# sashapersonxyz/Multi-camera_3D_Pose_Estimation

Measured on AMD Instinct MI355X. Metric: multi-view frames/sec end-to-end (2-cam HRNet-W32, 17 kpts) at 1/2/4/8 GPUs, higher is better.
Workload: dtype bf16; 1 GPU; BASELINE config 2: 2-cam HRNet-W32 256x192 bf16 (flip test) + batched 4x4 DLT-SVD triangulation; views=2, parallelism=dp1 (frame-sharded)

## Files before the change

### include/mvpose.h

```cpp
#ifndef MVPOSE_H
#define MVPOSE_H

#include <stddef.h>
#include <stdint.h>

#ifdef __cplusplus
extern "C" {
#endif

#define MVP_ABI_VERSION 1

#define MVP_OK 0
#define MVP_ERR_ARG (-1)
#define MVP_ERR_HIP (-2)
#define MVP_ERR_NOMEM (-3)
#define MVP_ERR_INTERNAL (-4)

int mvp_abi_version(void);
const char* mvp_last_error(void);

#define MVP_CAM_DOUBLES 40

int mvp_camera_pack(const double* K_host, const double* dist5_host, const double* R_host,
                    const double* T_host, double* out_record_host);
// ... 49 lines not shown

#define MVP_OP_STEM 0
#define MVP_OP_CONV 1
#define MVP_OP_FUSE 2

typedef struct mvp_tensor_desc {
    int h, w, c, dtype;
} mvp_tensor_desc;

typedef struct mvp_op_desc {
    int kind;
    int out;
    int n_in;
    int in[4];
    int up[4];
    int cin, cout, ks, stride, relu;
    int segment;
    int64_t w_off;
    int64_t b_off;
} mvp_op_desc;

int mvp_graph_create(const mvp_tensor_desc* tensors_host, int n_tensors, const mvp_op_desc* ops_host, int n_ops,
                     const int* seg_micro_batch_host, int n_segments, int input_tensor, int output_tensor,
                     const uint16_t* w_bf16_dev, int64_t w_elems, const float* f32_dev, int64_t f32_elems,
                     int max_batch, void** handle_out);
int mvp_graph_forward(void* handle, const void* input_dev, int batch, void* output_dev, void* stream);
int mvp_graph_arena_bytes(void* handle, int64_t* bytes_out);
int mvp_graph_refresh_weights(void* handle);
int mvp_graph_destroy(void* handle);
int mvp_graph_plan(void* handle, int batch, int64_t* rec_out, int max_records, int* n_records,
                   int64_t* covered_macs_out);
int mvp_graph_kernels(void* handle, int batch, int* kernels_out, int max_records, int* n_records);
const char* mvp_graph_kernel_name(int kernel);

#define MVP_DET_STEM 0
#define MVP_DET_CONV 1
#define MVP_DET_DW 2
#define MVP_DET_CA 3
#define MVP_DET_SPP 4
#define MVP_DET_UP2 5
#define MVP_DET_HEAD 6
#define MVP_DET_DWPW 7

typedef struct mvp_det_view {
    int t;
    int coff;
    int c;
} mvp_det_view;

typedef struct mvp_det_op {
    int kind;
    mvp_det_view in, out, res;
    int ks, stride, act;
    int64_t w_off, b_off;
    int64_t aux;
} mvp_det_op;

int mvp_det_letterbox(const uint8_t* frames_dev, int n, int h, int w, int size, const float* mean3_host,
                      const float* std3_host, void* out_dev, void* stream);
int mvp_det_create(const mvp_tensor_desc* tensors_host, int n_tensors, const mvp_det_op* ops_host, int n_ops,
                   int input_tensor, int size, int n_priors, const uint16_t* w_bf16_dev, int64_t w_elems,
                   const float* f32_dev, int64_t f32_elems, int max_batch, void** handle_out);
int mvp_det_forward(void* handle, const uint8_t* frames_dev, int n, int h, int w, float score_thr, float* cand_dev,
                    float* best_dev, void* letterboxed_dev, void* stream);
int mvp_det_nms(const float* cand_dev, int n, int n_priors, const int* level_off_host, int n_levels, int nms_pre,
                float score_thr, float iou_thr, int max_det, float fx, float fy, float* dets_dev, int* counts_dev,
// ... 147 lines not shown
```

### multi-camera_3d_pose_estimation_amd/csrc/conv.h

```cpp
#pragma once
#include <hip/hip_runtime.h>
#include <cstdint>

#include "kernel_select.h"
#include "mvp_common.h"

namespace mvp {

struct ConvLaunch {
    const uint16_t* x;
    const uint16_t* w;
    const float* bias;
    const uint16_t* res;
    uint16_t* y;
    float* yf;
    int N, H, W, Cin, Cout;
    int ks, stride, relu, out_f32_nchw;
    const uint16_t* x2 = nullptr;
    int c1 = 0;
    int x_stride = 0, y_stride = 0, r_stride = 0;
    const uint16_t* w_img = nullptr;
    int s2_tile = 0;
};


void launch_conv_generic(const ConvLaunch& c, hipStream_t s);

void launch_head1x1(const ConvLaunch& c, hipStream_t s);
bool head_fuse_supported(int cin, int cout, int n_in);
void launch_head_fuse(const uint16_t* const* in, const int* up, int n_in, int relu, const uint16_t* w,
                      const float* bias, float* y, int N, int H, int W, hipStream_t s);

void launch_conv1x1_direct(const ConvLaunch& c, hipStream_t s);
void launch_conv1x1_wide(const ConvLaunch& c, hipStream_t s);

struct PairLaunch {
    const uint16_t* x = nullptr;
    const uint16_t* x2 = nullptr;
    int c1 = 0, c2 = 0;
    const uint16_t* w1 = nullptr;
    const float* b1 = nullptr;
    const uint16_t* res = nullptr;
    uint16_t* y = nullptr;
    const uint16_t* w2 = nullptr;
    const float* b2 = nullptr;
    uint16_t* y2 = nullptr;
    long n_pix = 0;
};
bool conv1x1_pair_supported(int cin_total, int cmid, int cout2);
void launch_conv1x1_pair(const PairLaunch& p, hipStream_t s);


struct BneckLaunch {
    const uint16_t* x = nullptr;
    const uint16_t* w1 = nullptr;
    const float* b1 = nullptr;
    const uint16_t* w2 = nullptr;
    const float* b2 = nullptr;
    const uint16_t* w3 = nullptr;
    const float* b3 = nullptr;
    uint16_t* y = nullptr;
    int N = 0, H = 0, W = 0;
    int perm = 1;
    int lead = 0;
    int planar = 0;
};
bool bneck_supported(int H, int W, int C, int M);
void launch_bneck(const BneckLaunch& c, hipStream_t s);

void launch_tconv(const ConvLaunch& c, hipStream_t s);
void launch_tconv16(const ConvLaunch& c, hipStream_t s);
void tconv16_pack_weights(const uint16_t* w, uint16_t* img, int cin, int cout, hipStream_t s);

void launch_s2conv(const ConvLaunch& c, hipStream_t s);

struct S2Multi {
    const uint16_t* x = nullptr;
    const uint16_t* w = nullptr;
    const float* bias = nullptr;
    int N = 0, H = 0, W = 0, Cin = 0;
    int n_out = 0;
    uint16_t* y[3] = {nullptr, nullptr, nullptr};
    int cout[3] = {0, 0, 0};
    int relu[3] = {0, 0, 0};
};
bool s2conv_multi_supported(int H, int W, int Cin, int total_cout);
void launch_s2conv_multi(const S2Multi& m, hipStream_t s);

void launch_stem(const uint16_t* x, const float* w, const float* bias, uint16_t* y, int N, int H, int W,
                 hipStream_t s);

bool stem2_supported(int H, int W, int cin2, int cout2);
void launch_stem2(const uint16_t* x, const float* w1, const float* b1, const uint16_t* w2, const float* b2,
                  uint16_t* y, int N, int H, int W, bool crop_ranges, hipStream_t s);

bool trans1_supported(int H, int W, int C, int cout0, int cout1);
void launch_trans1(const uint16_t* x, const uint16_t* wimg, const float* b0, const float* b1, uint16_t* y0,
                   uint16_t* y1, int N, bool planar, hipStream_t s);
constexpr long kTrans1ImageElems = 16L * 9 * 2 * 96 * 8;
void trans1_pack_weights(const uint16_t* wb, int64_t w0_off, int64_t w1_off, uint16_t* img, hipStream_t s);

void launch_fuse_sum(const uint16_t* const* in, const int* up, int n_in, uint16_t* out, int N, int H, int W,
                     int C, int relu, hipStream_t s);

constexpr int kZeroSlots = 4096;
const uint16_t* conv_zero_region();
uint16_t* conv_sink_region();

template <auto Kern, int LDS, typename... Args>
void launch_lds(int grid, int threads, hipStream_t s, const Args&... args) {
    static const bool attr = [] {
        MVP_HIP(hipFuncSetAttribute((const void*)Kern, hipFuncAttributeMaxDynamicSharedMemorySize, LDS));
        return true;
    }();
    (void)attr;
    hipLaunchKernelGGL(Kern, dim3(grid), dim3(threads), LDS, s, args...);
}
// ... 14 lines not shown
```

### multi-camera_3d_pose_estimation_amd/csrc/graph.cpp

```cpp
#include <algorithm>
#include <cstdlib>
#include <cstring>
#include <vector>

#include "conv.h"
#include "mvp_common.h"

namespace mvp {
namespace {

struct Launch {
    Route route;
    int op;
    std::vector<int> covers;
    std::vector<int> reads;
    std::vector<int> writes;
    KernelChoice kernel;
    int64_t macs = 0;
    int cat_src = -1;
    int tail = -1;
    int conv1 = -1, conv2 = -1;
    int perm = 0;
    int lead = 0;
    int stem = -1;
// ... 24 lines not shown
    int cus = 0;
    std::vector<Launch> launches;
    std::vector<int> owner;
    std::vector<int64_t> offset;
    int64_t arena_bytes = 0;
    char* arena = nullptr;
};

int64_t elem_size(int dtype) { return dtype == MVP_DT_F32_NCHW ? 4 : 2; }

int64_t tensor_bytes(const mvp_tensor_desc& t, int batch) {
    return (int64_t)batch * t.h * t.w * t.c * elem_size(t.dtype);
}

Switches read_switches() {
    auto first_is = [](const char* name, char c) {
        const char* e = getenv(name);
        return e && e[0] == c;
    };
    Switches sw;
    sw.no_fuse = first_is("MVPOSE_NO_FUSE", '1');
    sw.no_catfuse = first_is("MVPOSE_NO_CATFUSE", '1');
    sw.no_pairfuse = first_is("MVPOSE_NO_PAIRFUSE", '1');
    sw.no_bneck = first_is("MVPOSE_NO_BNECK", '1');
    sw.no_stemfuse = first_is("MVPOSE_NO_STEMFUSE", '1');
    sw.no_transfuse = first_is("MVPOSE_NO_TRANSFUSE", '1');
    sw.no_sibfuse = first_is("MVPOSE_NO_SIBFUSE", '1');
    sw.no_headfuse = first_is("MVPOSE_NO_HEADFUSE", '1');
    sw.no_tblock64 = first_is("MVPOSE_NO_TBLOCK64", '1');
    sw.no_head1x1 = first_is("MVPOSE_NO_HEAD1X1", '1');
    sw.no_tconv = first_is("MVPOSE_NO_TCONV", '1');
    sw.no_tconv16 = first_is("MVPOSE_TCONV16", '0');
    sw.no_s2conv = first_is("MVPOSE_NO_S2CONV", '1');
    sw.no_tblock = first_is("MVPOSE_NO_TBLOCK", '1');
    sw.no_tblock32s = first_is("MVPOSE_NO_TBLOCK32S", '1');
    sw.stem2_tile = first_is("MVPOSE_STEM2_TILE", '1');
    sw.crop_stream = first_is("MVPOSE_CROP_STREAM", '1');
    const char* e = getenv("MVPOSE_S2_TILE");
    sw.s2_tile = e ? atoi(e) : 0;
    return sw;
}

void validate(Graph& g, int64_t w_elems, int64_t f_elems) {
    const int nt = (int)g.tensors.size();
    auto T = [&](int id) -> const mvp_tensor_desc& {
        MVP_REQUIRE(id >= 0 && id < nt, "graph: tensor id %d out of range", id);
        return g.tensors[id];
    };
    std::vector<int> defined(nt, 0);
    defined[g.input] = 1;
    for (size_t k = 0; k < g.ops.size(); k++) {
        const mvp_op_desc& op = g.ops[k];
        const mvp_tensor_desc& o = T(op.out);
        MVP_REQUIRE(op.n_in >= 1 && op.n_in <= 4, "graph op %zu: n_in=%d", k, op.n_in);
        for (int i = 0; i < op.n_in; i++) {
            if (op.kind == MVP_OP_CONV && i == 1 && op.in[1] < 0) continue;
            T(op.in[i]);
            MVP_REQUIRE(defined[op.in[i]], "graph op %zu reads tensor %d before it is produced", k, op.in[i]);
        }
        MVP_REQUIRE(!defined[op.out], "graph op %zu: tensor %d produced twice", k, op.out);
        if (op.kind == MVP_OP_STEM) {
            const mvp_tensor_desc& x = T(op.in[0]);
            MVP_REQUIRE(x.c == 4 && x.dtype == MVP_DT_BF16_NHWC, "stem: input must be bf16 NHWC with 4 channels");
            MVP_REQUIRE(o.c == 64 && o.h == (x.h - 1) / 2 + 1 && o.w == (x.w - 1) / 2 + 1, "stem: output shape");
            MVP_REQUIRE(op.w_off >= 0 && op.w_off + 64 * 36 <= f_elems && op.b_off >= 0 && op.b_off + 64 <= f_elems,
                        "stem: weights out of the f32 blob");
// ... 598 lines not shown
        const mvp_op_desc& op = g->ops[L.op];
        const mvp_tensor_desc& o = g->tensors[op.out];
        const mvp_tensor_desc& x = g->tensors[L.reads[0]];
        const mvp::Kernel kernel = mvp::pick_kernel(L.kernel, nb, g->cus, g->sw);
        switch (L.route) {
        case mvp::R_BLOCK: {
            const mvp_op_desc& c1 = g->ops[L.op - 1];
            const uint16_t *xb = bf16(op.in[1]), *w1 = g->wb + c1.w_off, *w2 = g->wb + op.w_off;
            const float *b1 = g->fb + c1.b_off, *b2 = g->fb + op.b_off;
            uint16_t* y = bf16(op.out);
            switch (kernel) {
            case mvp::K_TBLOCK32S: mvp::launch_tblock32s(xb, w1, b1, w2, b2, y, nb, o.h, o.w, s); break;
            case mvp::K_TBLOCK32: mvp::launch_tblock32(xb, w1, b1, w2, b2, y, nb, o.h, o.w, s); break;
            case mvp::K_BASIC_BLOCK_C32: mvp::launch_basic_block_c32(xb, w1, b1, w2, b2, y, nb, o.h, o.w, s); break;
            default: mvp::launch_tblock64(xb, w1, b1, w2, b2, y, nb, o.h, o.w, kernel == mvp::K_TBLOCK64, s);
            }
            break;
        }
        case mvp::R_TWIN: {
            const mvp_op_desc& b = g->ops[L.twin];
            mvp::launch_trans1(bf16(op.in[0]), L.w_img, g->fb + op.b_off, g->fb + b.b_off, bf16(op.out),
                               bf16(b.out), nb, L.planar, s);
            break;
        }
        case mvp::R_SIBLINGS: {
            mvp::S2Multi m;
            m.x = bf16(op.in[0]), m.w = L.w, m.bias = L.b;
            m.N = nb, m.H = x.h, m.W = x.w, m.Cin = op.cin;
            m.n_out = (int)L.covers.size();
            for (int i = 0; i < m.n_out; i++) {
                const mvp_op_desc& o2 = g->ops[L.covers[i]];
                m.y[i] = bf16(o2.out), m.cout[i] = o2.cout, m.relu[i] = o2.relu;
            }
            mvp::launch_s2conv_multi(m, s);
            break;
        }
        case mvp::R_HEAD_FUSE: {
            const mvp_op_desc& f = g->ops[L.fuse];
            const mvp_tensor_desc& fo = g->tensors[f.out];
            const uint16_t* ins[4];
            for (int i = 0; i < f.n_in; i++) ins[i] = bf16(f.in[i]);
            mvp::launch_head_fuse(ins, f.up, f.n_in, f.relu, g->wb + op.w_off, g->fb + op.b_off, (float*)ptr(op.out),
                                  nb, fo.h, fo.w, s);
            break;
        }
        case mvp::R_BNECK: {
            const mvp_op_desc& a = g->ops[L.conv1];
            const mvp_op_desc& c2 = g->ops[L.conv2];
            mvp::BneckLaunch bl;
            bl.x = bf16(a.in[0]);
            bl.w1 = g->wb + a.w_off, bl.b1 = g->fb + a.b_off;
            bl.w2 = g->wb + c2.w_off, bl.b2 = g->fb + c2.b_off;
            bl.w3 = L.lead ? L.w : g->wb + op.w_off, bl.b3 = L.lead ? L.b : g->fb + op.b_off;
            bl.y = bf16(op.out);
            bl.N = nb, bl.H = x.h, bl.W = x.w;
            bl.perm = L.perm, bl.lead = L.lead, bl.planar = L.planar;
            mvp::launch_bneck(bl, s);
            break;
        }
        case mvp::R_STEM2: {
            const mvp_op_desc& st = g->ops[L.stem];
            mvp::launch_stem2(bf16(st.in[0]), g->fb + st.w_off, g->fb + st.b_off, g->wb + op.w_off, g->fb + op.b_off,
                              bf16(op.out), nb, x.h, x.w, kernel == mvp::K_STEM2, s);
            break;
        }
        case mvp::R_STEM:
            mvp::launch_stem(bf16(op.in[0]), g->fb + op.w_off, g->fb + op.b_off, bf16(op.out), nb, x.h, x.w, s);
            break;
        case mvp::R_CONV:
        case mvp::R_PAIR: {
            mvp::ConvLaunch c{};
            c.x = bf16(op.in[0]);
            c.w = g->wb + op.w_off, c.bias = g->fb + op.b_off;
            c.res = mvp::has_res(op) ? bf16(op.in[1]) : nullptr;
            c.out_f32_nchw = o.dtype == MVP_DT_F32_NCHW;
            c.y = c.out_f32_nchw ? nullptr : bf16(op.out);
            c.yf = c.out_f32_nchw ? (float*)ptr(op.out) : nullptr;
            c.N = nb, c.H = x.h, c.W = x.w;
            c.Cin = op.cin, c.Cout = op.cout, c.ks = op.ks, c.stride = op.stride, c.relu = op.relu;
            c.w_img = L.w_img, c.s2_tile = g->sw.s2_tile;
            if (L.cat_src >= 0) {
                const mvp_op_desc& a = g->ops[L.cat_src];
                c.x2 = bf16(a.in[0]), c.c1 = op.cin, c.Cin = op.cin + a.cin;
                c.w = L.w, c.bias = L.b, c.res = nullptr;
            }
            if (L.route == mvp::R_CONV) {
                switch (kernel) {
                case mvp::K_HEAD1X1: mvp::launch_head1x1(c, s); break;
                case mvp::K_CONV1X1_WIDE: mvp::launch_conv1x1_wide(c, s); break;
                case mvp::K_CONV1X1: mvp::launch_conv1x1_direct(c, s); break;
                case mvp::K_TCONV: mvp::launch_tconv(c, s); break;
                case mvp::K_TCONV16: mvp::launch_tconv16(c, s); break;
                case mvp::K_S2CONV: mvp::launch_s2conv(c, s); break;
                default: mvp::launch_conv_generic(c, s);
                }
                break;
            }
            const mvp_op_desc& b = g->ops[L.tail];
            mvp::PairLaunch pl;
            pl.x = c.x, pl.x2 = c.x2;
            pl.c1 = c.x2 ? c.c1 : c.Cin, pl.c2 = c.x2 ? c.Cin - c.c1 : 0;
            pl.w1 = c.w, pl.b1 = c.bias, pl.res = c.res, pl.y = c.y;
            pl.w2 = g->wb + b.w_off, pl.b2 = g->fb + b.b_off, pl.y2 = bf16(b.out);
            pl.n_pix = (long)nb * x.h * x.w;
            mvp::launch_conv1x1_pair(pl, s);
            break;
        }
        case mvp::R_FUSE_SUM: {
            const uint16_t* ins[4];
            for (int i = 0; i < op.n_in; i++) ins[i] = bf16(op.in[i]);
            mvp::launch_fuse_sum(ins, op.up, op.n_in, bf16(op.out), nb, o.h, o.w, o.c, op.relu, s);
            break;
        }
// ... 14 lines not shown
    MVP_REQUIRE(batch > 0 && batch <= g->max_batch, "mvp_graph_plan: batch %d", batch);
    int n = 0;
    int64_t total = 0;
    mvp::for_each_micro_batch(*g, batch, [&](const mvp::Segment& sg, int64_t, int nb) {
        for (int l = sg.first_launch; l < sg.end_launch; l++, n++) {
            const Launch& L = g->launches[l];
            total += L.macs * nb;
            if (n >= max_records) continue;
            const int64_t rec[4] = {L.op, L.route, nb, L.macs * nb};
            std::copy(rec, rec + 4, rec_out + 4 * n);
        }
    });
    *n_records = n;
    if (covered_macs_out) *covered_macs_out = total;
    MVP_ABI_END
}

extern "C" int mvp_graph_kernels(void* handle, int batch, int* kernels_out, int max_records, int* n_records) {
    MVP_ABI_BEGIN
    Graph* g = static_cast<Graph*>(handle);
    MVP_REQUIRE(g && kernels_out && n_records, "mvp_graph_kernels: NULL pointer");
    MVP_REQUIRE(batch > 0 && batch <= g->max_batch, "mvp_graph_kernels: batch %d", batch);
    int n = 0;
    mvp::for_each_micro_batch(*g, batch, [&](const mvp::Segment& sg, int64_t, int nb) {
        for (int l = sg.first_launch; l < sg.end_launch; l++, n++)
            if (n < max_records) kernels_out[n] = mvp::pick_kernel(g->launches[l].kernel, nb, g->cus, g->sw);
    });
    *n_records = n;
    MVP_ABI_END
}

extern "C" const char* mvp_graph_kernel_name(int kernel) { return mvp::kernel_name(kernel); }

extern "C" int mvp_graph_refresh_weights(void* handle) {
    MVP_ABI_BEGIN
    Graph* g = static_cast<Graph*>(handle);
    MVP_REQUIRE(g != nullptr, "mvp_graph_refresh_weights: NULL handle");
    MVP_HIP(hipDeviceSynchronize());
    mvp::fill_weights(*g);
    MVP_ABI_END
}

extern "C" int mvp_graph_arena_bytes(void* handle, int64_t* bytes_out) {
    MVP_ABI_BEGIN
    MVP_REQUIRE(handle && bytes_out, "mvp_graph_arena_bytes: NULL argument");
    *bytes_out = static_cast<Graph*>(handle)->arena_bytes;
    MVP_ABI_END
}

extern "C" int mvp_graph_destroy(void* handle) {
    MVP_ABI_BEGIN
    Graph* g = static_cast<Graph*>(handle);
    if (g) {
        if (g->arena) (void)hipFree(g->arena);
        mvp::free_weights(*g);
        delete g;
    }
    MVP_ABI_END
}
```

### multi-camera_3d_pose_estimation_amd/csrc/kernel_select.h

```cpp
#pragma once

namespace mvp {

struct Switches {
    bool no_fuse = false;
    bool no_catfuse = false;
    bool no_pairfuse = false;
    bool no_bneck = false;
    bool no_stemfuse = false;
    bool no_transfuse = false;
    bool no_sibfuse = false;
    bool no_headfuse = false;
    bool no_tblock64 = false;
    bool no_head1x1 = false;
    bool no_tconv = false;
    bool no_tconv16 = false;
    bool no_s2conv = false;
    bool no_tblock = false;
    bool no_tblock32s = false;
    bool stem2_tile = false;
    bool crop_stream = false;
    int s2_tile = 0;
};

enum Route {
    R_BLOCK = 1,
    R_TWIN = 2,
    R_SIBLINGS = 3,
    R_HEAD_FUSE = 4,
    R_BNECK = 5,
    R_STEM2 = 6,
    R_STEM = 7,
    R_CONV = 8,
    R_PAIR = 9,
    R_FUSE_SUM = 10,
};

enum Kernel {
    K_NONE = 0,
    K_HEAD1X1,
    K_CONV1X1_WIDE,
    K_CONV1X1,
    K_TCONV,
    K_TCONV16,
    K_S2CONV,
    K_CONV_MFMA,
    K_TBLOCK32S,
    K_TBLOCK32,
    K_BASIC_BLOCK_C32,
    K_TBLOCK64,
// ... 68 lines not shown
    if (plane && c.stride == 2 && !c.res && !sw.no_s2conv) {
        if (c.h == 64 && c.w == 48 && c.cout == 64 && c.cin == 32) return K_S2CONV;
        if (c.h == 32 && c.w == 24 && c.cout == 128 && (c.cin == 32 || c.cin == 64)) return K_S2CONV;
        if (s2conv_streams_image(c)) return K_S2CONV;
    }
    return K_CONV_MFMA;
}

inline KernelChoice select_kernel(Route route, const LaunchShape& c, const Switches& sw, bool has_image) {
    auto one = [](Kernel k) { return KernelChoice{k, k}; };
    switch (route) {
    case R_CONV: return one(select_conv(c, sw, has_image));
    case R_BLOCK: {
        if (c.cin == 64) return {K_TBLOCK64_TILES, K_TBLOCK64};
        const Kernel tile = c.w == 48 && c.h % 16 == 0 && !sw.no_tblock ? K_TBLOCK32 : K_BASIC_BLOCK_C32;
        const bool s32 = c.h == 64 && c.w == 48 && !sw.no_tblock32s && !sw.no_tblock;
        return {tile, s32 ? K_TBLOCK32S : tile};
    }
    case R_STEM2: return {K_STEM2_TILE, sw.stem2_tile ? K_STEM2_TILE : K_STEM2};
    case R_STEM: {
        const int ho = (c.h - 1) / 2 + 1, wo = (c.w - 1) / 2 + 1;
        return one(wo == 96 && c.h % 2 == 0 && ho % 2 == 0 ? K_STEM_MFMA : K_STEM);
    }
    case R_TWIN: return one(K_TRANS1);
    case R_SIBLINGS: return one(K_S2CONV_MULTI);
    case R_HEAD_FUSE: return one(K_HEAD_FUSE);
    case R_BNECK: return one(K_BNECK);
    case R_PAIR: return one(K_CONV1X1_PAIR);
    case R_FUSE_SUM: return one(K_FUSE_SUM);
    }
    return {};
}

inline long conv_image_elems(Kernel k, const LaunchShape& c) {
    return k == K_TCONV16 || (k == K_S2CONV && s2conv_streams_image(c)) ? (long)c.cout * 9 * c.cin : 0;
}

}
```

### multi-camera_3d_pose_estimation_amd/csrc/s2conv.hip

```cpp
#include <algorithm>
#include <cstdlib>

#include "conv.h"
#include "mfma_tile.h"
#include "mvp_common.h"

namespace mvp {
namespace {

using namespace mfma_tile;

template <int CIN, int H, int W, int TH, int NB, bool WRES, int BM>
struct SCfg {
    static constexpr int NW = 8, NT_THREADS = NW * 64;
    static constexpr int MG = BM / 32, PG = NW / MG;
    static constexpr int NT = 3;
    static constexpr int HO = H / 2, WO = W / 2;
    static constexpr int P = NB * TH * WO;
    static constexpr int NCH = CIN / 16;
    static constexpr int RS = WO + 1, HR = TH + 1;
    static constexpr int PH = HR * RS;
    static constexpr int HS = NB * 4 * PH;
    static constexpr int HT = 2 * HS;
    static constexpr int QS = 1, PS = 2;
    static constexpr int WT = 9 * 2 * BM;
    static constexpr int ITEM_SLOTS = HT + (WRES ? 0 : WT);
    static constexpr int PPW = (ITEM_SLOTS + 64 * NW - 1) / (64 * NW);
    static constexpr int BUF = PPW * NW * 1024;
    static constexpr int WPPW = WRES ? (NCH * WT + 64 * NW - 1) / (64 * NW) : 0;
    static constexpr int WOFF = 2 * BUF;
    static constexpr int LDS = 2 * BUF + WPPW * NW * 1024;
    static constexpr int STORES = 2 * NT;
    static_assert(P == PG * NT * 32, "tile = pixel groups x 3 fragments x 32 pixels");
    static_assert(H % 2 == 0 && W % 2 == 0 && HO % TH == 0 && CIN % 16 == 0, "tiling");
    static_assert(LDS <= 160 * 1024, "LDS budget");
    static_assert((QS + (3 * PH + RS + 1) * PS) * 16 < 65536 && (16 * BM + 2 * BM) * 16 < 65536,
                  "ds_read offset range");
    static_assert(STORES < 64 && 2 * PPW < 64, "vmcnt range");
// ... 150 lines not shown
            const int cur = tap & 1;
            if (tap + 1 < 9) load(tap + 1, fa[cur ^ 1], fb[cur ^ 1]);
            __builtin_amdgcn_sched_barrier(0);
#pragma unroll
            for (int t = 0; t < G::NT; t++)
                acc[t] = __builtin_amdgcn_mfma_f32_32x32x16_bf16(fa[cur], fb[cur][t], acc[t], 0, 0, 0);
            __builtin_amdgcn_sched_barrier(0);
        }

        if (last) {
            const long pix0 = (long)(n0 * G::HO + ho0) * G::WO;
            uint16_t* yb = p.y;
            int cs = p.Cout, cl = cob, rl = p.relu;
            bool cok = true;
            if (cob >= p.Cout) {
                const bool s1 = cob < p.Cout + p.c1;
                yb = s1 ? p.y1 : p.y2;
                cs = s1 ? p.c1 : p.c2;
                cl = s1 ? cob - p.Cout : cob - p.Cout - p.c1;
                rl = s1 ? p.relu1 : p.relu2;
                cok = cob < p.Cout + p.c1 + p.c2;
            }
#pragma unroll
            for (int t = 0; t < G::NT; t++) {
                const bool ok = n0 + enb[t] < p.N && cok;
                uint16_t* yrow = ok ? yb + (pix0 + eoff[t]) * cs + cl : p.sink + lane * 16;
                store_row16(yrow, pack_row16(acc[t], rl != 0));
            }
        }
    }
    asm volatile("s_waitcnt vmcnt(0)" ::: "memory");
}

template <int CIN, int H, int W, int TH, int NB, bool WRES, int BM>
void launch_sp(const SParams& p, hipStream_t s) {
    using G = SCfg<CIN, H, W, TH, NB, WRES, BM>;
    const int grid = std::min(p.n_tiles, cu_count());
    launch_lds<s2conv_kernel<CIN, H, W, TH, NB, WRES, BM>, G::LDS>(grid, G::NT_THREADS, s, p);
}

template <int CIN, int H, int W, int TH, int NB, bool WRES, int BM>
void launch_s(const ConvLaunch& c, hipStream_t s) {
    using G = SCfg<CIN, H, W, TH, NB, WRES, BM>;
    MVP_REQUIRE(!WRES || c.Cout == BM, "s2conv: resident weights need Cout == BM");
    MVP_REQUIRE(c.Cout % BM == 0, "s2conv: Cout %d not a multiple of %d", c.Cout, BM);
    MVP_REQUIRE(c.Cin == CIN && c.H == H && c.W == W, "s2conv: plane mismatch");
    const long tiles = (long)((c.N + NB - 1) / NB) * (G::HO / TH) * (c.Cout / BM);
    MVP_REQUIRE(tiles < (1L << 30), "s2conv: too many tiles");
    const bool img = !WRES && BM == 128 && c.w_img != nullptr;
    SParams p{c.x, img ? c.w_img : c.w, c.bias, c.y, conv_zero_region(), conv_sink_region(), c.N, c.Cout, (int)tiles,
              c.Cout / BM, c.relu, nullptr, nullptr, 0, 0, 0, 0, img ? 1 : 0};
    launch_sp<CIN, H, W, TH, NB, WRES, BM>(p, s);
}

}

bool s2conv_multi_supported(int H, int W, int Cin, int total_cout) {
    return H == 64 && W == 48 && Cin == 32 && total_cout <= 128;
}

void launch_s2conv_multi(const S2Multi& m, hipStream_t s) {
    MVP_REQUIRE(m.n_out >= 1 && m.n_out <= 3, "s2conv_multi: %d outputs", m.n_out);
    int tot = 0;
    for (int i = 0; i < m.n_out; i++) {
        MVP_REQUIRE(m.cout[i] % 32 == 0 && m.cout[i] > 0, "s2conv_multi: cout %d", m.cout[i]);
        tot += m.cout[i];
    }
    MVP_REQUIRE(s2conv_multi_supported(m.H, m.W, m.Cin, tot), "s2conv_multi: unsupported plane");
    using G = SCfg<32, 64, 48, 8, 1, true, 128>;
    const long tiles = (long)m.N * (G::HO / 8);
    SParams p{m.x, m.w, m.bias, m.y[0], conv_zero_region(), conv_sink_region(), m.N, m.cout[0], (int)tiles, 1, m.relu[0],
              m.n_out > 1 ? m.y[1] : nullptr, m.n_out > 2 ? m.y[2] : nullptr, m.n_out > 1 ? m.cout[1] : 0,
              m.n_out > 2 ? m.cout[2] : 0, m.n_out > 1 ? m.relu[1] : 0, m.n_out > 2 ? m.relu[2] : 0, 0};
    if (tiles == 0) return;
    launch_sp<32, 64, 48, 8, 1, true, 128>(p, s);
    MVP_HIP(hipGetLastError());
}

void launch_s2conv(const ConvLaunch& c, hipStream_t s) {
    MVP_REQUIRE(c.ks == 3 && c.stride == 2 && !c.out_f32_nchw && !c.res && !c.x2, "s2conv: not a plain 3x3/s2 conv");
    const int ci = c.Cin, co = c.Cout, h = c.H, w = c.W;
    const bool p24 = h == 32 && w == 24 && co == 128;
    const bool p12 = h == 16 && w == 12 && co % 128 == 0;
    if (h == 64 && w == 48 && co == 64 && ci == 32)
        launch_s<32, 64, 48, 16, 1, true, 64>(c, s);
    else if (p24 && ci == 32)
        launch_s<32, 32, 24, 16, 1, true, 128>(c, s);
    else if (p24 && ci == 64)
        launch_s<64, 32, 24, 16, 1, false, 128>(c, s);
    else if (p12 && ci == 32)
        launch_s<32, 16, 12, 8, 4, false, 128>(c, s);
    else if (p12 && ci == 64)
        launch_s<64, 16, 12, 8, 4, false, 128>(c, s);
    else if (p12 && ci == 128)
        launch_s<128, 16, 12, 8, 4, false, 128>(c, s);
    else
        fail(MVP_ERR_ARG, "s2conv: unsupported plane %d -> %d @ %dx%d", ci, co, h, w);
    MVP_HIP(hipGetLastError());
}

}
```

### multi-camera_3d_pose_estimation_amd/mvpose/_lib.py

```python
from __future__ import annotations

import ctypes
import os

_HERE = os.path.dirname(os.path.abspath(__file__))
LIB_PATH = os.environ.get("MVPOSE_LIB", os.path.join(_HERE, "libmvpose.so"))


class MvposeError(RuntimeError):

    def __init__(self, fn: str, code: int, msg: str):
        super().__init__(f"{fn} failed (code {code}): {msg}")
        self.code = code


if not os.path.exists(LIB_PATH):
    raise ImportError(
        f"libmvpose.so not found at {LIB_PATH}: build it with "
        "`make -C multi-camera_3d_pose_estimation_amd` (or __graft_entry__.build()). "
        "There is no CPU fallback.")

lib = ctypes.CDLL(LIB_PATH)

c_int, c_int64, c_float, c_double, c_void_p, c_size_t = (
# ... 13 lines not shown
                                       c_int, c_void_p, c_int, c_float, c_float, c_int, c_double, c_void_p,
                                       c_void_p, c_void_p, c_void_p, c_void_p]),
    "mvp_triangulate_points_f64": (c_int, [c_void_p, c_int64, c_void_p, c_void_p, c_void_p, c_void_p]),
    "mvp_triangulate_fallback_total": (c_int, [c_void_p, P(ctypes.c_ulonglong)]),
    "mvp_mp4v_create": (c_int, [c_void_p, c_size_t, P(c_void_p), P(c_int), P(c_int)]),
    "mvp_mp4v_decode": (c_int, [c_void_p, c_void_p, c_size_t, c_void_p, c_void_p, P(c_int)]),
    "mvp_mp4v_destroy": (c_int, [c_void_p]),
    "mvp_mp4v_selfcheck": (c_int, []),
    "mvp_mp4v_parse": (c_int, [c_void_p, c_void_p, c_size_t, c_void_p, c_int64, c_void_p, c_int64, P(c_int64),
                               P(c_int)]),
    "mvp_mp4v_reconstruct": (c_int, [c_void_p, c_int, c_int, c_int, c_void_p]),
    "mvp_mp4v_parse_many": (c_int, [c_void_p, c_int, c_void_p, c_void_p, c_void_p, c_void_p, c_int64, c_void_p,
                                    c_void_p, P(c_int)]),
    "mvp_preprocess": (c_int, [c_void_p, c_int, c_int, c_int, c_void_p, c_int, c_int, P(c_float), P(c_float),
                               c_int, c_int, c_void_p, c_void_p]),
    "mvp_heatmap_decode": (c_int, [c_void_p, c_void_p, c_int, c_int, c_int, c_int, P(c_int), c_int, c_void_p,
                                   c_int, c_int, c_void_p, c_void_p, c_void_p, c_void_p, c_void_p, c_int,
                                   c_void_p]),
    "mvp_warp_is_separable": (c_int, [P(c_double), c_int, c_int, P(c_int)]),
    "mvp_heatmap_revert": (c_int, [c_void_p, c_int, c_int, c_int, c_int, c_void_p, c_int, c_int, c_void_p,
                                   c_void_p]),
    "mvp_heatmap_moments": (c_int, [c_void_p, c_int, c_int, c_int, c_int, c_void_p, c_int, c_int, c_float,
                                    c_int, c_void_p, c_void_p, c_void_p]),
    "mvp_bbox_geometry": (c_int, [c_void_p, c_int, c_int, c_int, c_float, c_int, c_int, c_void_p, c_void_p,
                                  c_void_p, c_void_p, c_void_p]),
    "mvp_graph_create": (c_int, None),
    "mvp_graph_forward": (c_int, [c_void_p, c_void_p, c_int, c_void_p, c_void_p]),
    "mvp_graph_arena_bytes": (c_int, None),
    "mvp_graph_refresh_weights": (c_int, [c_void_p]),
    "mvp_graph_destroy": (c_int, [c_void_p]),
    "mvp_graph_plan": (c_int, [c_void_p, c_int, c_void_p, c_int, P(c_int), P(c_int64)]),
    "mvp_graph_kernels": (c_int, [c_void_p, c_int, c_void_p, c_int, P(c_int)]),
    "mvp_graph_kernel_name": (c_char_p, [c_int]),
    "mvp_det_letterbox": (c_int, [c_void_p, c_int, c_int, c_int, c_int, P(c_float), P(c_float), c_void_p,
                                  c_void_p]),
    "mvp_det_create": (c_int, None),
    "mvp_det_forward": (c_int, [c_void_p, c_void_p, c_int, c_int, c_int, c_float, c_void_p, c_void_p, c_void_p,
                                c_void_p]),
    "mvp_det_nms": (c_int, [c_void_p, c_int, c_int, P(c_int), c_int, c_int, c_float, c_float, c_int, c_float,
                            c_float, c_void_p, c_void_p, c_void_p]),
    "mvp_det_arena_bytes": (c_int, None),
    "mvp_det_run_ops": (c_int, [c_void_p, c_void_p, c_int, c_int, c_int, c_int, c_int, c_void_p, c_void_p]),
    "mvp_det_tensor_copy": (c_int, [c_void_p, c_int, c_int, c_void_p, c_int, c_void_p]),
    "mvp_det_folded_ops": (c_int, [c_void_p, c_void_p, c_int]),
    "mvp_det_kernels": (c_int, [c_void_p, c_void_p, c_int, P(c_int)]),
    "mvp_det_kernel_name": (c_char_p, [c_int]),
    "mvp_det_destroy": (c_int, [c_void_p]),
    "mvp_sgd_workspace_floats": (c_int, [c_int, c_int, c_int, c_int, P(c_int64)]),
    "mvp_sgd_refine": (c_int, None),
    "mvp_sgd_refine_cams": (c_int, None),
    "mvp_extrinsic_sample_grad": (c_int, [c_void_p, c_void_p, c_int, c_int64, c_void_p, c_int, c_int, c_void_p,
                                          c_void_p]),
    "mvp_extrinsic_adam_step": (c_int, [c_void_p, c_int, c_void_p, c_void_p, c_double, c_double, c_double, c_double,
                                        c_double, c_void_p, c_void_p, c_void_p]),
    "mvp_project_points": (c_int, [c_void_p, c_int64, c_void_p, c_int, c_void_p, c_void_p]),
    "mvp_linear_interpolation": (c_int, [c_void_p, c_int, c_int, c_int, c_int, c_float, c_float, c_int, c_int,
                                         c_void_p, c_void_p]),
    "mvp_trajectory_smooth_plan": (c_int, [c_int, c_int, c_int, P(c_int), P(c_int), P(c_int64)]),
    "mvp_trajectory_smooth": (c_int, [c_void_p, c_void_p, c_void_p, c_int, c_int, c_double, c_float, c_float, c_int,
                                      c_void_p, c_int64, c_void_p, c_void_p, c_void_p, c_void_p, c_void_p]),
    "mvp_trajectory_smooth_cov_plan": (c_int, [c_int, c_int, c_int, P(c_int), P(c_int), P(c_int64)]),
    "mvp_trajectory_smooth_cov": (c_int, [c_void_p, c_void_p, c_void_p, c_int, c_int, c_double, c_float, c_float,
                                          c_int, c_void_p, c_int64, c_void_p, c_void_p, c_void_p, c_void_p]),
    "mvp_epipolar_lag_cost_plan": (c_int, [c_int, c_int, c_int, c_int, P(c_int), P(c_int64)]),
    "mvp_epipolar_lag_cost": (c_int, [c_void_p, c_int, c_int, c_int, c_void_p, c_int, P(c_int), c_int, c_int, c_float,
                                      c_float, c_void_p, c_int64, c_void_p, c_void_p, c_void_p]),
# ... 59 lines not shown
```

### multi-camera_3d_pose_estimation_amd/mvpose/hrnet.py

```python
from __future__ import annotations

import ctypes
import os

import numpy as np
import torch

from . import _lib
from ._lib import call

BN_EPS = 1e-5
STAGES = ((1, (32, 64)), (4, (32, 64, 128)), (3, (32, 64, 128, 256)))
N_JOINTS = 17
INPUT_HW = (256, 192)
HEATMAP_HW = (64, 48)
DT_BF16, DT_F32 = 0, 1
OP_STEM, OP_CONV, OP_FUSE = 0, 1, 2


class TensorDesc(ctypes.Structure):
    _fields_ = [("h", ctypes.c_int), ("w", ctypes.c_int), ("c", ctypes.c_int), ("dtype", ctypes.c_int)]


class OpDesc(ctypes.Structure):
# ... 504 lines not shown
        world, _ = mdist.world_rank()
        if world > 1:
            mdist.broadcast_([self.w_dev, self.f_dev], src=src)
            torch.cuda.synchronize(self.device)
            self.refresh_weights()

    @property
    def arena_bytes(self) -> int:
        b = ctypes.c_int64()
        call("mvp_graph_arena_bytes", self._h, ctypes.byref(b))
        return b.value

    def launch_plan(self, batch: int) -> np.ndarray:
        cap = 4096
        rec = np.zeros((cap, 4), np.int64)
        n, tot = ctypes.c_int(), ctypes.c_int64()
        call("mvp_graph_plan", self._h, int(batch), ctypes.c_void_p(rec.ctypes.data), cap, ctypes.byref(n),
             ctypes.byref(tot))
        if n.value > cap:
            raise RuntimeError(f"{n.value} launches > {cap}")
        rec = rec[:n.value].copy()
        assert int(rec[:, 3].sum()) == tot.value == self.macs_per_crop() * batch
        return rec

    def launch_kernels(self, batch: int) -> list[str]:
        cap = 4096
        ids = np.zeros(cap, np.int32)
        n = ctypes.c_int()
        call("mvp_graph_kernels", self._h, int(batch), ctypes.c_void_p(ids.ctypes.data), cap, ctypes.byref(n))
        if n.value > cap:
            raise RuntimeError(f"{n.value} launches > {cap}")
        return [_lib.lib.mvp_graph_kernel_name(int(k)).decode() for k in ids[:n.value]]

    def macs_per_crop(self) -> int:
        macs = 0
        for op in self.spec.ops:
            if op["kind"] in (OP_STEM, OP_CONV):
                h, w, _, _ = self.spec.tensors[op["out"]]
                cin = 3 if op["kind"] == OP_STEM else op["cin"]
                macs += h * w * op["cout"] * cin * op["ks"] ** 2
        return macs

    def close(self):
        if getattr(self, "_h", None):
            call("mvp_graph_destroy", self._h)
            self._h = None

    def __del__(self):
        try:
            self.close()
        except Exception:
            pass


class HRNetBackbone(ConvGraph):

    def __init__(self, state_dict=None, seed: int = 0, max_batch: int = 256, device="cuda", micro_batch=None):
        if state_dict is None:
            state_dict = random_state_dict(seed)
        spec, input_id, output_id = build_hrnet_w32(state_dict, micro_batch)
        super().__init__(spec, input_id, output_id, max_batch, device)

    def forward(self, crops: torch.Tensor, out: torch.Tensor | None = None) -> torch.Tensor:
        if crops.dtype != torch.bfloat16 or not crops.is_cuda or not crops.is_contiguous():
            raise ValueError("crops must be a contiguous bf16 CUDA tensor (N,256,192,4)")
        if tuple(crops.shape[1:]) != (INPUT_HW[0], INPUT_HW[1], 4):
# ... 8 lines not shown
```

Measured before the change: 13040 frames/s.

## Add halo-tiled persistent stride-2 conv kernel with double-buffered LDS staging

```diff
diff --git a/include/mvpose.h b/include/mvpose.h
--- a/include/mvpose.h
+++ b/include/mvpose.h
@@ -105,6 +105,7 @@
                    int64_t* covered_macs_out);
 int mvp_graph_kernels(void* handle, int batch, int* kernels_out, int max_records, int* n_records);
 const char* mvp_graph_kernel_name(int kernel);
+int mvp_graph_s2conv_forms(void* handle, int batch, int* forms_out, int max_records, int* n_records);
 
 #define MVP_DET_STEM 0
 #define MVP_DET_CONV 1
diff --git a/multi-camera_3d_pose_estimation_amd/csrc/conv.h b/multi-camera_3d_pose_estimation_amd/csrc/conv.h
--- a/multi-camera_3d_pose_estimation_amd/csrc/conv.h
+++ b/multi-camera_3d_pose_estimation_amd/csrc/conv.h
@@ -21,6 +21,7 @@
     int x_stride = 0, y_stride = 0, r_stride = 0;
     const uint16_t* w_img = nullptr;
     int s2_tile = 0;
+    int s2_items = 0;
 };
 
 
@@ -83,6 +84,7 @@
     uint16_t* y[3] = {nullptr, nullptr, nullptr};
     int cout[3] = {0, 0, 0};
     int relu[3] = {0, 0, 0};
+    int items = 0;
 };
 bool s2conv_multi_supported(int H, int W, int Cin, int total_cout);
 void launch_s2conv_multi(const S2Multi& m, hipStream_t s);
diff --git a/multi-camera_3d_pose_estimation_amd/csrc/graph.cpp b/multi-camera_3d_pose_estimation_amd/csrc/graph.cpp
--- a/multi-camera_3d_pose_estimation_amd/csrc/graph.cpp
+++ b/multi-camera_3d_pose_estimation_amd/csrc/graph.cpp
@@ -80,6 +80,7 @@
     sw.no_tconv = first_is("MVPOSE_NO_TCONV", '1');
     sw.no_tconv16 = first_is("MVPOSE_TCONV16", '0');
     sw.no_s2conv = first_is("MVPOSE_NO_S2CONV", '1');
+    sw.s2conv_items = first_is("MVPOSE_S2CONV_ITEMS", '1');
     sw.no_tblock = first_is("MVPOSE_NO_TBLOCK", '1');
     sw.no_tblock32s = first_is("MVPOSE_NO_TBLOCK32S", '1');
     sw.stem2_tile = first_is("MVPOSE_STEM2_TILE", '1');
@@ -744,6 +745,7 @@
                 const mvp_op_desc& o2 = g->ops[L.covers[i]];
                 m.y[i] = bf16(o2.out), m.cout[i] = o2.cout, m.relu[i] = o2.relu;
             }
+            m.items = g->sw.s2conv_items;
             mvp::launch_s2conv_multi(m, s);
             break;
         }
@@ -790,7 +792,7 @@
             c.yf = c.out_f32_nchw ? (float*)ptr(op.out) : nullptr;
             c.N = nb, c.H = x.h, c.W = x.w;
             c.Cin = op.cin, c.Cout = op.cout, c.ks = op.ks, c.stride = op.stride, c.relu = op.relu;
-            c.w_img = L.w_img, c.s2_tile = g->sw.s2_tile;
+            c.w_img = L.w_img, c.s2_tile = g->sw.s2_tile, c.s2_items = g->sw.s2conv_items;
             if (L.cat_src >= 0) {
                 const mvp_op_desc& a = g->ops[L.cat_src];
                 c.x2 = bf16(a.in[0]), c.c1 = op.cin, c.Cin = op.cin + a.cin;
@@ -871,6 +873,23 @@
 
 extern "C" const char* mvp_graph_kernel_name(int kernel) { return mvp::kernel_name(kernel); }
 
+extern "C" int mvp_graph_s2conv_forms(void* handle, int batch, int* forms_out, int max_records, int* n_records) {
+    MVP_ABI_BEGIN
+    Graph* g = static_cast<Graph*>(handle);
+    MVP_REQUIRE(g && forms_out && n_records, "mvp_graph_s2conv_forms: NULL pointer");
+    MVP_REQUIRE(batch > 0 && batch <= g->max_batch, "mvp_graph_s2conv_forms: batch %d", batch);
+    int n = 0;
+    mvp::for_each_micro_batch(*g, batch, [&](const mvp::Segment& sg, int64_t, int nb) {
+        for (int l = sg.first_launch; l < sg.end_launch; l++, n++) {
+            if (n >= max_records) continue;
+            const Launch& L = g->launches[l];
+            forms_out[n] = mvp::s2conv_form(mvp::pick_kernel(L.kernel, nb, g->cus, g->sw), mvp::launch_shape(*g, L), g->sw);
+        }
+    });
+    *n_records = n;
+    MVP_ABI_END
+}
+
 extern "C" int mvp_graph_refresh_weights(void* handle) {
     MVP_ABI_BEGIN
     Graph* g = static_cast<Graph*>(handle);
diff --git a/multi-camera_3d_pose_estimation_amd/csrc/kernel_select.h b/multi-camera_3d_pose_estimation_amd/csrc/kernel_select.h
--- a/multi-camera_3d_pose_estimation_amd/csrc/kernel_select.h
+++ b/multi-camera_3d_pose_estimation_amd/csrc/kernel_select.h
@@ -16,6 +16,7 @@
     bool no_tconv = false;
     bool no_tconv16 = false;
     bool no_s2conv = false;
+    bool s2conv_items = false;
     bool no_tblock = false;
     bool no_tblock32s = false;
     bool stem2_tile = false;
@@ -150,6 +151,23 @@
     return {};
 }
 
+enum S2Form {
+    S2_NONE = 0,
+    S2_ITEMS = 1,
+    S2_HALO = 2,
+};
+
+inline bool s2conv_halo_plane(int cin, int cout, int h, int w) {
+    if (h == 64 && w == 48) return cin == 32 && (cout == 64 || cout == 128);
+    return h == 32 && w == 24 && cout == 128 && cin == 32;
+}
+
+inline S2Form s2conv_form(Kernel k, const LaunchShape& c, const Switches& sw) {
+    if (k != K_S2CONV && k != K_S2CONV_MULTI) return S2_NONE;
+    if (sw.s2conv_items) return S2_ITEMS;
+    return s2conv_halo_plane(c.cin, k == K_S2CONV_MULTI ? 128 : c.cout, c.h, c.w) ? S2_HALO : S2_ITEMS;
+}
+
 inline long conv_image_elems(Kernel k, const LaunchShape& c) {
     return k == K_TCONV16 || (k == K_S2CONV && s2conv_streams_image(c)) ? (long)c.cout * 9 * c.cin : 0;
 }
diff --git a/multi-camera_3d_pose_estimation_amd/csrc/s2conv.hip b/multi-camera_3d_pose_estimation_amd/csrc/s2conv.hip
--- a/multi-camera_3d_pose_estimation_amd/csrc/s2conv.hip
+++ b/multi-camera_3d_pose_estimation_amd/csrc/s2conv.hip
@@ -4,6 +4,7 @@
 #include "conv.h"
 #include "mfma_tile.h"
 #include "mvp_common.h"
+#include "s2conv_halo.h"
 
 namespace mvp {
 namespace {
@@ -220,6 +221,157 @@
     asm volatile("s_waitcnt vmcnt(0)" ::: "memory");
 }
 
+template <int H_, int W_, int TH_>
+struct HCfg {
+    static constexpr int CIN = 32, H = H_, W = W_, TH = TH_, BM = 128;
+    static constexpr int NW = 8, NT_THREADS = NW * 64, MG = 4, PG = 2, NT = 3;
+    static constexpr int HO = H / 2, WO = W / 2, P = TH * WO;
+    using HL = s2halo::Halo<W, TH>;
+    static constexpr int LPR = W / 2;
+    static constexpr int PPW = (HL::PIECES + NW - 1) / NW;
+    static constexpr int ZOFF = HL::SLOTS * 16;
+    static constexpr int BUF = ZOFF + 512;
+    static constexpr int BIAS = 2 * BUF;
+    static constexpr int LDS = 2 * BUF + 512;
+    static constexpr int STORES = 2 * NT;
+    static_assert(P == PG * NT * 32 && HO % TH == 0 && WO <= 24, "tile = 2 pixel groups x 3 fragments x 32 pixels");
+    static_assert(LDS <= 160 * 1024 && BUF + 1024 < 65536, "LDS budget, ds_read offset range (buffer 1 + tap)");
+};
+
+template <class G>
+__global__ __launch_bounds__(512, 1) void s2conv_kernel(SParams p) {
+    constexpr int CIN = G::CIN, H = G::H, W = G::W, TH = G::TH;
+    extern __shared__ __attribute__((aligned(1024))) uint8_t lds[];
+    const int tid = threadIdx.x, lane = tid & 63, h = lane >> 5, r32 = lane & 31;
+    const int wave = __builtin_amdgcn_readfirstlane(tid >> 6);
+    const int mg = wave % G::MG, pg = wave / G::MG;
+    if ((int)blockIdx.x >= p.n_tiles) return;
+    constexpr int tiles_h = G::HO / TH;
+    const int cob = mg * 32 + 16 * h;
+    const int couts = p.Cout + p.c1 + p.c2;
+    const bool live = mg * 32 < couts;
+
+    bf16x8 wreg[18];
+    if (live) {
+        const uint16_t* wl = p.w + (long)(mg * 32 + row_cout(r32)) * 9 * CIN + h * 8;
+#pragma unroll
+        for (int st = 0; st < 18; st++)
+            wreg[st] = *reinterpret_cast<const bf16x8*>(wl + (st % 9) * CIN + (st / 9) * 16);
+    } else {
+#pragma unroll
+        for (int st = 0; st < 18; st++) wreg[st] = bf16x8{};
+    }
+    if (tid < 128) reinterpret_cast<float*>(lds + G::BIAS)[tid] = tid < couts ? p.bias[tid] : 0.f;
+    if (tid < 64) *reinterpret_cast<uint4*>(lds + (tid >> 5) * G::BUF + G::ZOFF + (tid & 31) * 16) = uint4{0, 0, 0, 0};
+#pragma unroll
+    for (int st = 0; st < 18; st++) asm volatile("" : "+v"(wreg[st]));
+    asm volatile("s_waitcnt lgkmcnt(0)" ::: "memory");
+
+    const int lsrc = s2halo::lane_src_bytes(lane), lline = lane & 7;
+    const uint8_t* zl = reinterpret_cast<const uint8_t*>(p.zero) + lane * 16;
+    auto issue = [&](int k, int buf) {
+        const int tile = blockIdx.x + k * gridDim.x;
+        const int n0 = tile / tiles_h, ho0 = (tile - n0 * tiles_h) * TH;
+        const uint8_t* xb = reinterpret_cast<const uint8_t*>(p.x) + ((long)(n0 * H + 2 * ho0 - 1) * W) * (2 * CIN) + lsrc;
+        const int top = ho0 == 0 ? G::LPR : 0;
+        uint8_t* dst = lds + buf * G::BUF;
+#pragma unroll
+        for (int j = 0; j < G::PPW; j++) {
+            const int pc = j * G::NW + wave;
+            const int line = pc * 8 + lline;
+            const uint8_t* src = line >= top && line < G::HL::LINES ? xb + pc * 1024 : zl;
+            if (j < G::PPW - 1 || pc < G::HL::PIECES) glds16(src, dst + s2halo::piece_slot(pc) * 16);
+        }
+    };
+
+    int bv[G::NT][3][2], eoff[G::NT];
+#pragma unroll
+    for (int t = 0; t < G::NT; t++) {
+        int g2;
+        const int rank = lane_rank(r32, g2);
+        const int pp = (2 * (pg * G::NT + t) + g2) * 16 + rank;
+        const int ty = pp / G::WO, x = pp - ty * G::WO;
+#pragma unroll
+        for (int dy = 0; dy < 3; dy++) {
+            bv[t][dy][0] = x == 0 ? G::ZOFF + h * 128 : s2halo::pixel_slot<W>(2 * ty + dy, 2 * x - 1, h) * 16;
+            bv[t][dy][1] = s2halo::pixel_slot<W>(2 * ty + dy, 2 * x, h) * 16;
+        }
+        eoff[t] = pp;
+    }
+
+    const int n_my = (p.n_tiles - 1 - (int)blockIdx.x) / (int)gridDim.x + 1;
+    issue(0, 0);
+    for (int k = 0; k < n_my; k++) {
+        const int buf = k & 1;
+        if (k == 0 || !live)
+            asm volatile("s_waitcnt vmcnt(0)" ::: "memory");
+        else
+            asm volatile("s_waitcnt vmcnt(%0)" ::"n"(G::STORES) : "memory");
+        asm volatile("" ::: "memory");
+        __builtin_amdgcn_s_barrier();
+        asm volatile("" ::: "memory");
+        if (k + 1 < n_my) issue(k + 1, buf ^ 1);
+        asm volatile("" ::: "memory");
+        if (!live) continue;
+
+        f32x16 acc[G::NT];
+        {
+            const f32x16 b = load_f32x16(reinterpret_cast<const float*>(lds + G::BIAS) + cob);
+#pragma unroll
+            for (int t = 0; t < G::NT; t++) acc[t] = b;
+        }
+        auto steps = [&](auto bc) {
+            constexpr int B = decltype(bc)::value;
+            auto load = [&](int st, bf16x8 (&b)[G::NT]) {
+                const int slice = st / 9, tap = st % 9, dy = tap / 3, dx = tap % 3;
+                const int off = B * G::BUF + slice * 256 + (dx == 2 ? 512 : 0);
+#pragma unroll
+                for (int t = 0; t < G::NT; t++)
+                    b[t] = *reinterpret_cast<const bf16x8*>(lds + bv[t][dy][dx ? 1 : 0] + off);
+            };
+            bf16x8 fb[2][G::NT];
+            load(0, fb[0]);
+#pragma unroll
+            for (int st = 0; st < 18; st++) {
+                const int cur = st & 1;
+                if (st + 1 < 18) load(st + 1, fb[cur ^ 1]);
+                __builtin_amdgcn_sched_barrier(0);
+#pragma unroll
+                for (int t = 0; t < G::NT; t++)
+                    acc[t] = __builtin_amdgcn_mfma_f32_32x32x16_bf16(wreg[st], fb[cur][t], acc[t], 0, 0, 0);
+                __builtin_amdgcn_sched_barrier(0);
+            }
+        };
+        if (buf == 0)
+            steps(std::integral_constant<int, 0>{});
+        else
+            steps(std::integral_constant<int, 1>{});
+
+        const int tile = blockIdx.x + k * gridDim.x;
+        const int n0 = tile / tiles_h, ho0 = (tile - n0 * tiles_h) * TH;
+        const long pix0 = (long)(n0 * G::HO + ho0) * G::WO;
+        uint16_t* yb = p.y;
+        int cs = p.Cout, cl = cob, rl = p.relu;
+        if (cob >= p.Cout) {
+            const bool s1 = cob < p.Cout + p.c1;
+            yb = s1 ? p.y1 : p.y2;
+            cs = s1 ? p.c1 : p.c2;
+            cl = s1 ? cob - p.Cout : cob - p.Cout - p.c1;
+            rl = s1 ? p.relu1 : p.relu2;
+        }
+#pragma unroll
+        for (int t = 0; t < G::NT; t++) store_row16(yb + (pix0 + eoff[t]) * cs + cl, pack_row16(acc[t], rl != 0));
+    }
+    asm volatile("s_waitcnt vmcnt(0)" ::: "memory");
+}
+
+template <class G>
+void launch_halo(const SParams& p, hipStream_t s) {
+    if (p.n_tiles == 0) return;
+    const int grid = std::min(p.n_tiles, cu_count());
+    launch_lds<s2conv_kernel<G>, G::LDS>(grid, G::NT_THREADS, s, p);
+}
+
 template <int CIN, int H, int W, int TH, int NB, bool WRES, int BM>
 void launch_sp(const SParams& p, hipStream_t s) {
     using G = SCfg<CIN, H, W, TH, NB, WRES, BM>;
@@ -261,7 +413,10 @@
               m.n_out > 1 ? m.y[1] : nullptr, m.n_out > 2 ? m.y[2] : nullptr, m.n_out > 1 ? m.cout[1] : 0,
               m.n_out > 2 ? m.cout[2] : 0, m.n_out > 1 ? m.relu[1] : 0, m.n_out > 2 ? m.relu[2] : 0, 0};
     if (tiles == 0) return;
-    launch_sp<32, 64, 48, 8, 1, true, 128>(p, s);
+    if (m.items)
+        launch_sp<32, 64, 48, 8, 1, true, 128>(p, s);
+    else
+        launch_halo<HCfg<64, 48, 8>>(p, s);
     MVP_HIP(hipGetLastError());
 }
 
@@ -270,12 +425,28 @@
     const int ci = c.Cin, co = c.Cout, h = c.H, w = c.W;
     const bool p24 = h == 32 && w == 24 && co == 128;
     const bool p12 = h == 16 && w == 12 && co % 128 == 0;
-    if (h == 64 && w == 48 && co == 64 && ci == 32)
-        launch_s<32, 64, 48, 16, 1, true, 64>(c, s);
-    else if (p24 && ci == 32)
-        launch_s<32, 32, 24, 16, 1, true, 128>(c, s);
-    else if (p24 && ci == 64)
+    const bool halo = !c.s2_items && s2conv_halo_plane(ci, co, h, w);
+    auto launch_h = [&](auto cfg) {
+        using G = decltype(cfg);
+        const long tiles = (long)c.N * (G::HO / G::TH);
+        MVP_REQUIRE(tiles < (1L << 30), "s2conv: too many tiles");
+        launch_halo<G>(SParams{c.x, c.w, c.bias, c.y, conv_zero_region(), conv_sink_region(), c.N, c.Cout, (int)tiles, 1,
+                               c.relu, nullptr, nullptr, 0, 0, 0, 0, 0},
+                       s);
+    };
+    if (h == 64 && w == 48 && co == 64 && ci == 32) {
+        if (halo)
+            launch_h(HCfg<64, 48, 8>{});
+        else
+            launch_s<32, 64, 48, 16, 1, true, 64>(c, s);
+    } else if (p24 && ci == 32) {
+        if (halo)
+            launch_h(HCfg<32, 24, 16>{});
+        else
+            launch_s<32, 32, 24, 16, 1, true, 128>(c, s);
+    } else if (p24 && ci == 64) {
         launch_s<64, 32, 24, 16, 1, false, 128>(c, s);
+    }
     else if (p12 && ci == 32)
         launch_s<32, 16, 12, 8, 4, false, 128>(c, s);
     else if (p12 && ci == 64)
diff --git a/multi-camera_3d_pose_estimation_amd/csrc/s2conv_halo.h b/multi-camera_3d_pose_estimation_amd/csrc/s2conv_halo.h
--- /dev/null
+++ b/multi-camera_3d_pose_estimation_amd/csrc/s2conv_halo.h
@@ -0,0 +1,33 @@
+#pragma once
+
+namespace mvp {
+namespace s2halo {
+
+constexpr int kPieceSlots = 72;
+constexpr int kSuperSlots = 220;
+constexpr int kSuperLines = 24;
+
+constexpr int lane_src_bytes(int lane) {
+    const int line = lane & 7, sub = lane >> 3;
+    return line * 128 + (sub >> 2) * 64 + (sub & 3) * 16;
+}
+
+constexpr int piece_slot(int pc) { return (pc / 3) * kSuperSlots + (pc % 3) * kPieceSlots; }
+
+template <int W>
+constexpr int pixel_slot(int r, int c, int q) {
+    static_assert(W == 48 || W == 24, "a super-row is one or two input rows");
+    const int line = r * (W / 2) + (c >> 1);
+    const int s = line / kSuperLines, m = line - s * kSuperLines;
+    return s * kSuperSlots + (m >> 3) * kPieceSlots + ((c & 1) * 4 + q) * 8 + (m & 7);
+}
+
+template <int W, int TH>
+struct Halo {
+    static constexpr int LINES = (2 * TH + 1) * (W / 2);
+    static constexpr int PIECES = (LINES + 7) / 8;
+    static constexpr int SLOTS = ((PIECES + 2) / 3) * kSuperSlots;
+};
+
+}
+}
diff --git a/multi-camera_3d_pose_estimation_amd/mvpose/_lib.py b/multi-camera_3d_pose_estimation_amd/mvpose/_lib.py
--- a/multi-camera_3d_pose_estimation_amd/mvpose/_lib.py
+++ b/multi-camera_3d_pose_estimation_amd/mvpose/_lib.py
@@ -69,6 +69,7 @@
     "mvp_graph_plan": (c_int, [c_void_p, c_int, c_void_p, c_int, P(c_int), P(c_int64)]),
     "mvp_graph_kernels": (c_int, [c_void_p, c_int, c_void_p, c_int, P(c_int)]),
     "mvp_graph_kernel_name": (c_char_p, [c_int]),
+    "mvp_graph_s2conv_forms": (c_int, [c_void_p, c_int, c_void_p, c_int, P(c_int)]),
     "mvp_det_letterbox": (c_int, [c_void_p, c_int, c_int, c_int, c_int, P(c_float), P(c_float), c_void_p,
                                   c_void_p]),
     "mvp_det_create": (c_int, None),
diff --git a/multi-camera_3d_pose_estimation_amd/mvpose/hrnet.py b/multi-camera_3d_pose_estimation_amd/mvpose/hrnet.py
--- a/multi-camera_3d_pose_estimation_amd/mvpose/hrnet.py
+++ b/multi-camera_3d_pose_estimation_amd/mvpose/hrnet.py
@@ -560,6 +560,17 @@
             raise RuntimeError(f"{n.value} launches > {cap}")
         return [_lib.lib.mvp_graph_kernel_name(int(k)).decode() for k in ids[:n.value]]
 
+    S2CONV_FORMS = ("", "items", "halo")
+
+    def s2conv_forms(self, batch: int) -> list[str]:
+        cap = 4096
+        ids = np.zeros(cap, np.int32)
+        n = ctypes.c_int()
+        call("mvp_graph_s2conv_forms", self._h, int(batch), ctypes.c_void_p(ids.ctypes.data), cap, ctypes.byref(n))
+        if n.value > cap:
+            raise RuntimeError(f"{n.value} launches > {cap}")
+        return [self.S2CONV_FORMS[int(k)] for k in ids[:n.value]]
+
     def macs_per_crop(self) -> int:
         macs = 0
         for op in self.spec.ops:
```

After: 13140 frames/s, median of 6. No clear change (+0.7%).
